# rajashree-srikanth/drone-sim-python

Hardware: NVIDIA B200
Metric: closed-loop aircraft-steps/s (higher is better)
Workload: dtype f64

## Files before the change

drone-sim-python_b200/csrc/d2dx_api.cu:

```cuda
#include <math.h>
#include <string.h>

#include "d2dx_device.cuh"
#include "d2dx_host.h"

namespace d2dx {

static thread_local char g_err[512] = "";

int set_error(int code, const char* fmt, ...) {
  va_list ap;
  va_start(ap, fmt);
  vsnprintf(g_err, sizeof(g_err), fmt, ap);
  va_end(ap);
  return code;
}

int rollout_resident_threads_per_sm();
int formation_resident_threads_per_sm();
int colloc_resident_threads_per_sm();

constexpr int kThreads = 128;
inline int grid_for(long n) { return (int)((n + kThreads - 1) / kThreads); }

// ... 82 lines not shown
  Ur[i] = r.u_phi; Ur[(size_t)n + i] = r.u_v;
  if (Xd) {
    Xd[i] = 0.0; Xd[(size_t)n + i] = 0.0; Xd[2 * (size_t)n + i] = r.psidot; Xd[3 * (size_t)n + i] = 0.0; Xd[4 * (size_t)n + i] = r.vadot;
  }
}

__global__ void __launch_bounds__(kThreads) dfff_control_kernel(const d2dx_traj_table tt, const double* __restrict__ X, double t,
                                                                 const double* __restrict__ W, const double* __restrict__ ac,
                                                                 const d2dx_dfff_gains g, double* __restrict__ U,
                                                                 double* __restrict__ Xr, double* __restrict__ K,
                                                                 double* __restrict__ care_state) {
  const int B = tt.n_traj, S = tt.n_seg;
  const int b = blockIdx.x * kThreads + threadIdx.x;
  if (b >= B) return;
  double te;
  const int seg = composite_locate(tt, b, t, te);
  auto P = [&](int k) { return tt.seg_par[(size_t)k * S + seg]; };
  FlatOut Y;
  segment_eval<false>(tt.seg_type[seg], P, te, Y, &tt);
  const AcPar a = load_ac(W, ac, B, b);
  double x[5];
  for (int k = 0; k < 5; ++k) x[k] = X[(size_t)k * B + b];
  const CareConst cc = care_const(g);
  CareState cs = {0.0, 1.0, 1.0, 0.0, 0.0};
  bool cold = true;
  if (care_state) {
    cs.C = care_state[b]; cs.S = care_state[B + b]; cs.al = care_state[2 * (size_t)B + b];
    cs.dth = care_state[3 * (size_t)B + b]; cs.dal = care_state[4 * (size_t)B + b];
    cold = !(cs.al > 0.0);
  }
  int flags = 0;
  RefCtl rc;
  double u_phi, u_v;
  make_ref(Y, a, ac[B + b], cc, cs, cold, flags, rc);
  feedback(rc, x, g, u_phi, u_v);
  U[b] = u_phi; U[(size_t)B + b] = u_v;
  if (Xr) { Xr[b] = rc.xr; Xr[(size_t)B + b] = rc.yr; Xr[2 * (size_t)B + b] = rc.psir; Xr[3 * (size_t)B + b] = rc.phir; Xr[4 * (size_t)B + b] = rc.var; }
  if (K) for (int k = 0; k < 6; ++k) K[(size_t)k * B + b] = rc.k[k];
  if (care_state) {
    care_state[b] = cs.C; care_state[B + b] = cs.S; care_state[2 * (size_t)B + b] = cold ? 0.0 : cs.al;
    care_state[3 * (size_t)B + b] = cs.dth; care_state[4 * (size_t)B + b] = cs.dal;
  }
}

__global__ void dfma_burn_kernel(int iters, double* sink) {
  double a[16];
  const double x = 1.0 + 1e-9 * threadIdx.x, y = 1e-12 * (blockIdx.x + 1);
#pragma unroll
  for (int k = 0; k < 16; ++k) a[k] = k * 0.5;
  for (int it = 0; it < iters; ++it) {
#pragma unroll
    for (int k = 0; k < 16; ++k) a[k] = fma(a[k], x, y);
  }
  double s = 0.0;
#pragma unroll
  for (int k = 0; k < 16; ++k) s += a[k];
  if (s == 123.456) *sink = s;
}

__global__ void math_probe_kernel(int n, const double* __restrict__ x, const double* __restrict__ y, double* __restrict__ out) {
  const int i = blockIdx.x * kThreads + threadIdx.x;
  if (i >= n) return;
  double s, c;
  fm::sincos(x[i], s, c);
// ... 160 lines not shown
```

drone-sim-python_b200/csrc/d2dx_device.cuh:

```cuda
#pragma once
#include <cuda_runtime.h>
#include <math.h>
#include <stdint.h>
#include <string.h>

#include "../../include/d2dx.h"
#include "d2dx_math.cuh"

namespace d2dx {

#ifdef D2DX_USE_LIBM
__device__ __forceinline__ void sincos_b(double x, double& s, double& c) { ::sincos(x, &s, &c); }
__device__ __forceinline__ void sincos_any(double x, double& s, double& c) { ::sincos(x, &s, &c); }
__device__ __forceinline__ double atan2_f(double y, double x) { return ::atan2(y, x); }
__device__ __forceinline__ double atan_f(double v) { return ::atan(v); }
__host__ __device__ __forceinline__ double sqrt_f(double v) { return ::sqrt(v); }
__host__ __device__ __forceinline__ double rsqrt_f(double v) { return 1.0 / ::sqrt(v); }
__host__ __device__ __forceinline__ double rcp_f(double v) { return 1.0 / v; }
__host__ __device__ __forceinline__ double div_f(double a, double b) { return a / b; }
#else
__device__ __forceinline__ void sincos_b(double x, double& s, double& c) { fm::sincos(x, s, c); }
struct SinCos { double s, c; };
static __device__ __noinline__ SinCos sincos_slow(double x) { SinCos r; ::sincos(x, &r.s, &r.c); return r; }
__device__ __forceinline__ void sincos_any(double x, double& s, double& c) {
// ... 332 lines not shown
  const double inv_va = rsqrt_f(va2), va = va2 * inv_va;
  r.x = Y.y0x; r.y = Y.y0y; r.va = va; r.inv_va = inv_va;
  r.psi = atan2_f(vay, vax);
  r.vadot = (vax * Y.y2x + vay * Y.y2y) * inv_va;
  const double num = Y.y2y * vax - Y.y2x * vay;
  r.psidot = num * inv_va * inv_va;
  r.z = num * inv_va * (1.0 / kG);
  r.phi = atan_f(r.z);
  r.u_phi = r.phi;
  r.u_v = tau_v * r.vadot + va;
  r.cpsi = vax * inv_va; r.spsi = vay * inv_va;
}

__host__ __device__ __forceinline__ int hi_word(double x) {
#ifdef __CUDA_ARCH__
  return __double2hiint(x);
#else
  long long b;
  memcpy(&b, &x, sizeof(b));
  return (int)(b >> 32);
#endif
}

struct CareState { double C, S, al, dth, dal; };

struct CareConst { double sq, q3, sr1, sr2, isr1, isr2; };

__host__ __device__ __forceinline__ CareConst care_const(const d2dx_dfff_gains& g) {
  CareConst c;
  c.sq = ::sqrt(g.q_pos); c.q3 = g.q_psi; c.sr1 = ::sqrt(g.r_phi); c.sr2 = ::sqrt(g.r_v);
  c.isr1 = 1.0 / c.sr1; c.isr2 = 1.0 / c.sr2;
  return c;
}

struct CareStep { double k1, ba, vc2, ve, k2, q3; };

__host__ __device__ __forceinline__ void care_residual(const CareStep& k, double C, double S, double al, double& be, double& F1, double& F2) {
  be = fma(k.k1, C, k.ba * al);
  F1 = fma(C, al, fma(S, be, fma(k.vc2, C, k.ve * S)));
  F2 = fma(al, al, fma(be, be, -fma(k.k2, S, k.q3)));
}

__host__ __device__ __forceinline__ void care_update(double& C, double& S, double& al, double dth, double dal) {
  const double Cn = fma(-S, dth, C), Sn = fma(C, dth, S);
  const double nrm = fma(-0.5, fma(Cn, Cn, Sn * Sn), 1.5);
  C = Cn * nrm; S = Sn * nrm; al += dal;
}

struct CareRoot { double C, S, al; bool conv; };
static __host__ __device__ __noinline__ CareRoot care_newton_loop_v(const CareStep k, double C, double S, double al, int max_it) {
  bool conv = false;
  for (int it = 0; it < max_it && !conv; ++it) {
    double be, F1, F2;
    care_residual(k, C, S, al, be, F1, F2);
    const double bt = -k.k1 * S;
    const double J11 = fma(-S, al, fma(C, be, fma(S, bt, fma(k.ve, C, -k.vc2 * S)))), J12 = fma(S, k.ba, C);
    const double J21 = 2.0 * fma(be, bt, -0.5 * k.k2 * C), J22 = 2.0 * fma(be, k.ba, al);
    const double idet = rcp_f(fma(J11, J22, -J12 * J21));
    const double dth = fma(J12, F2, -F1 * J22) * idet, dal = fma(J21, F1, -J11 * F2) * idet;
    const double Cn = C - S * dth, Sn = S + C * dth;
    const double nrm = rsqrt_f(fma(Cn, Cn, Sn * Sn));
    C = Cn * nrm; S = Sn * nrm; al += dal;
    conv = fabs(dth) < 3e-8 && fabs(dal) < 3e-8 * fabs(al);
  }
  CareRoot r;
  r.C = C; r.S = S; r.al = al; r.conv = conv;
  return r;
}
__host__ __device__ __forceinline__ bool care_newton_loop(const CareStep& k, double& C, double& S, double& al, int max_it) {
  const CareRoot r = care_newton_loop_v(k, C, S, al, max_it);
  C = r.C; S = r.S; al = r.al;
  return r.conv;
}

__host__ __device__ __forceinline__ bool care_gain(const CareConst& cc, double v, double c1, double e, CareState& st, bool cold, double* K0) {
  const double c1q = c1 * cc.sq;
  CareStep k;
  k.k1 = c1q * cc.isr2; k.ba = e * cc.isr2; k.vc2 = v * cc.sr2; k.ve = v * e; k.k2 = 2.0 * v * c1q; k.q3 = cc.q3;
  const double C0 = st.C, S0 = st.S, al0 = st.al;
  double C = C0, S = S0, al = al0;
  care_update(C, S, al, st.dth, st.dal);
  double be_, F1, F2;
  care_residual(k, C, S, al, be_, F1, F2);
  const double bt = -k.k1 * S;
  const double J11 = fma(-S, al, fma(C, be_, fma(S, bt, fma(k.ve, C, -k.vc2 * S)))), J12 = fma(S, k.ba, C);
  const double J21 = 2.0 * fma(be_, bt, -0.5 * k.k2 * C), J22 = 2.0 * fma(be_, k.ba, al);
  const double idet = rcp_f(fma(J11, J22, -J12 * J21));
  const double i11 = J22 * idet, i12 = -J12 * idet, i21 = -J21 * idet, i22 = J11 * idet;
  double dth = -fma(i11, F1, i12 * F2), dal = -fma(i21, F1, i22 * F2);
  care_update(C, S, al, dth, dal);
  care_residual(k, C, S, al, be_, F1, F2);
  dth = -fma(i11, F1, i12 * F2); dal = -fma(i21, F1, i22 * F2);
  care_update(C, S, al, dth, dal);
  bool ok = !cold && (hi_word(dth) & 0x7fffffff) < 0x3E601B2B && fabs(dal) < 3e-8 * fabs(al) && hi_word(S) > 0 && hi_word(al) > 0;
  if (!ok) {
    if (!cold) {
      C = C0; S = S0; al = al0;
      ok = care_newton_loop(k, C, S, al, 40) && S > 0.0 && al > 0.0;
    }
    if (!ok) { C = 0.0; S = 1.0; al = sqrt_f(cc.q3 + k.k2); ok = care_newton_loop(k, C, S, al, 60); }
  }
  st.dth = fma(C0, S, -S0 * C); st.dal = al - al0;
  if (cold || !((hi_word(st.dth) & 0x7fffffff) < 0x3F947AE1 && fabs(st.dal) < 0.02 * al)) { st.dth = 0.0; st.dal = 0.0; }
  st.C = C; st.S = S; st.al = al;
  const double be = fma(k.k1, C, k.ba * al);
  K0[0] = cc.sq * C * cc.isr1; K0[1] = cc.sq * S * cc.isr1; K0[2] = al * cc.isr1;
  K0[3] = cc.sq * S * cc.isr2; K0[4] = -cc.sq * C * cc.isr2; K0[5] = be * cc.isr2;
  return ok;
}

struct RefCtl { double xr, yr, psir, phir, var, uphi, uv, k[6]; };

__device__ __forceinline__ void make_ref(const FlatOut& Y, const AcPar& a, double tau_v, const CareConst& cc, CareState& cs,
                                         bool& cold, int& flags, RefCtl& r) {
  FlatState fr;
  flatness(Y, a.wx, a.wy, tau_v, fr);
  const double z2 = fr.z * fr.z;
  const double c1 = cc.sr1 * (2.0 + z2) * rcp_f(kG * fr.inv_va * (1.0 + z2));
  const double e = kG * fr.inv_va * fr.inv_va * fr.z * c1;
  double K0[6];
  if (care_gain(cc, fr.va, c1, e, cs, cold, K0)) cold = false;
  else { flags |= 2; cold = true; }
  r.xr = fr.x; r.yr = fr.y; r.psir = fr.psi; r.phir = fr.phi; r.var = fr.va; r.uphi = fr.u_phi; r.uv = fr.u_v;
#pragma unroll
  for (int m = 0; m < 2; ++m) {
    r.k[3 * m + 0] = K0[3 * m] * fr.cpsi - K0[3 * m + 1] * fr.spsi;
    r.k[3 * m + 1] = K0[3 * m] * fr.spsi + K0[3 * m + 1] * fr.cpsi;
    r.k[3 * m + 2] = K0[3 * m + 2];
  }
}

__device__ __forceinline__ void feedback(const RefCtl& r, const double* X, const d2dx_dfff_gains& g, double& u_phi, double& u_v) {
  const double ex = clip_sym(X[0] - r.xr, g.err_sat[0]);
  const double ey = clip_sym(X[1] - r.yr, g.err_sat[1]);
  const double ep = clip_sym(wrap_pi(X[2] - r.psir), g.err_sat[2]);
  u_phi = clip(r.uphi - fma(r.k[0], ex, fma(r.k[1], ey, r.k[2] * ep)), g.u_lo[0], g.u_hi[0]);
  u_v = clip(r.uv - fma(r.k[3], ex, fma(r.k[4], ey, r.k[5] * ep)), g.u_lo[1], g.u_hi[1]);
}

__device__ __forceinline__ void gvf_control(double px, double py, double psi, double v, double cx, double cy,
                                            double r, double ke, double kd, double& U, double& U1, double& U2) {
  const double dx = px - cx, dy = py - cy;
  const double e = (dx * dx + dy * dy) - r * r;
  const double nx = 2.0 * dx, ny = 2.0 * dy;
  double s, c;
  sincos_b(psi, s, c);
  const double pdx = v * c, pdy = v * s;
  const double tx = ny, ty = -nx;
  const double qx = tx - ke * e * nx, qy = ty - ke * e * ny;
  const double inrm = rsqrt_f(qx * qx + qy * qy);
  const double qnx = qx * inrm, qny = qy * inrm;
  const double ox = qny, oy = -qnx;
// ... 38 lines not shown
```

drone-sim-python_b200/csrc/d2dx_lqr5.cuh:

```cuda
#pragma once
#include "d2dx_device.cuh"

namespace d2dx {

struct Lqr5State { double C, S, p23, p24, p33, p34, p44; };

struct Lqr5Par { double v, a, b, itp, itv, s1, s2, i1, i2, sq, q3, q4, q5; };

__host__ __device__ __forceinline__ bool solve6(double (&J)[6][6], double (&F)[6], double (&d)[6]) {
  constexpr int perm[6] = {2, 0, 3, 1, 4, 5};
  double A[6][7];
#pragma unroll
  for (int i = 0; i < 6; ++i) {
#pragma unroll
    for (int j = 0; j < 6; ++j) A[i][j] = J[perm[i]][j];
    A[i][6] = -F[perm[i]];
  }
  bool ok = true;
#pragma unroll
  for (int k = 0; k < 6; ++k) {
    double amax = fabs(A[k][k]);
#pragma unroll
    for (int j = k + 1; j < 6; ++j) amax = fabs(A[k][j]) > amax ? fabs(A[k][j]) : amax;
    ok = ok && (fabs(A[k][k]) > 1e-9 * amax);
// ... 50 lines not shown
    J[3][4] = (sq * S + P.b * y2) * P.i2 * ia - x2 * P.i1; J[4][4] = -(P.itp + P.itv) - (x3 * P.i1 + y4 * P.i2); J[5][4] = -2.0 * x4 * P.i1;
    J[0][5] = 0.0; J[1][5] = 0.0; J[2][5] = sq * C * P.i2; J[3][5] = -y2 * P.i2; J[4][5] = -y3 * P.i2; J[5][5] = -2.0 * (P.itv + y4 * P.i2);
    if (!solve6(J, F, d)) return false;
    const double Cn = C - S * d[0], Sn = S + C * d[0];
    const double nrm = rsqrt_f(Cn * Cn + Sn * Sn);
    u.C = Cn * nrm; u.S = Sn * nrm;
    u.p23 += d[1]; u.p24 += d[2]; u.p33 += d[3]; u.p34 += d[4]; u.p44 += d[5];
    const double scale = fabs(u.p23) + fabs(u.p24) + fabs(u.p33) + fabs(u.p34) + fabs(u.p44);
    const double step = fabs(d[1]) + fabs(d[2]) + fabs(d[3]) + fabs(d[4]) + fabs(d[5]);
    if (fabs(d[0]) < 3e-8 && step < 3e-8 * scale) return true;
  }
  return false;
}

__host__ __device__ inline bool lqr5_gain(const Lqr5Par& P, double sr1, double sr2, double tau_phi, double tau_v, double r1, double r2,
                                          Lqr5State& st, double* Kp) {
  bool ok = false;
  if (st.p23 > 0.0) {
    Lqr5State w = st;
    ok = lqr5_newton(P, w, 12) && w.S > 0.0 && w.p23 > 0.0;
    if (ok) st = w;
  }
  if (!ok) {
    CareConst cc; cc.sq = P.sq; cc.q3 = P.q3; cc.sr1 = sr1; cc.sr2 = sr2; cc.isr1 = 1.0 / sr1; cc.isr2 = 1.0 / sr2;
    CareState c3 = {0.0, 1.0, 1.0, 0.0, 0.0};
    double K0[6];
    const double c1 = sr1 * rcp_f(P.a), e = P.b * c1;
    care_gain(cc, P.v, c1, e, c3, true, K0);
    const double al3 = K0[2] * sr1, be3 = K0[5] * sr2;
    st.C = c3.C; st.S = c3.S;
    st.p23 = P.s1 * al3; st.p24 = P.s2 * be3;
    st.p33 = tau_phi * (P.a * st.p23 + 0.5 * P.q4);
    st.p44 = tau_v * (P.s2 * P.sq * st.S + P.b * st.p24 + 0.5 * P.q5);
    st.p34 = (P.a * st.p24 + P.s1 * P.sq * st.C + P.b * st.p23) * rcp_f(P.itp + P.itv);
    ok = lqr5_newton(P, st, 40);
  }
  const double f1 = 1.0 / (tau_phi * r1), f2 = 1.0 / (tau_v * r2);
  Kp[0] = P.s1 * P.sq * st.C * f1; Kp[1] = P.s1 * P.sq * st.S * f1;
  Kp[5] = P.s2 * P.sq * st.S * f2; Kp[6] = -P.s2 * P.sq * st.C * f2;
  Kp[2] = st.p23 * f1; Kp[3] = st.p33 * f1; Kp[4] = st.p34 * f1;
  Kp[7] = st.p24 * f2; Kp[8] = st.p34 * f2; Kp[9] = st.p44 * f2;
  return ok;
}

}
```

drone-sim-python_b200/csrc/d2dx_rollout.cu:

```cuda
#include "d2dx_device.cuh"
#include "d2dx_host.h"

namespace d2dx {

constexpr int kRolloutThreads = 128;
#ifndef D2DX_ROLLOUT_MIN_BLOCKS
#define D2DX_ROLLOUT_MIN_BLOCKS 4
#endif

struct RolloutArgs {
  d2dx_scenarios s;
  d2dx_rollout_out o;
  d2dx_dfff_gains g;
  CareConst cc;
  const double* time;
  int i_begin, i_end, nsub, final_control;
};

__device__ __forceinline__ void tma_load_1d(void* smem_dst, const void* gmem_src, uint32_t bytes, uint64_t* bar) {
  const uint32_t dst = static_cast<uint32_t>(__cvta_generic_to_shared(smem_dst));
  const uint32_t mb = static_cast<uint32_t>(__cvta_generic_to_shared(bar));
  asm volatile("cp.async.bulk.shared::cluster.global.mbarrier::complete_tx::bytes [%0], [%1], %2, [%3];"
               :: "r"(dst), "l"(gmem_src), "r"(bytes), "r"(mb) : "memory");
}
// ... 38 lines not shown
      }
      mbar_wait(&bar, 0);
    } else {
      for (int k = 0; k < kRows; ++k) spar[k][tid] = tt.seg_par[(size_t)k * S + b];
    }
    cur_seg = b;
  }
  auto P = [&](int k) { return spar[k][tid]; };

  spar[D2DX_SEG_NPAR + 0][tid] = a.s.wind[b]; spar[D2DX_SEG_NPAR + 1][tid] = a.s.wind[B + b];
  spar[D2DX_SEG_NPAR + 2][tid] = -1.0 / a.s.ac[b]; spar[D2DX_SEG_NPAR + 3][tid] = -1.0 / a.s.ac[B + b];
  spar[D2DX_SEG_NPAR + 4][tid] = a.s.ac[B + b];
  auto load_ac = [&]() {
    AcPar ap;
    ap.wx = spar[D2DX_SEG_NPAR + 0][tid]; ap.wy = spar[D2DX_SEG_NPAR + 1][tid];
    ap.n_inv_tau_phi = spar[D2DX_SEG_NPAR + 2][tid]; ap.n_inv_tau_v = spar[D2DX_SEG_NPAR + 3][tid];
    return ap;
  };
  double X[5];
#pragma unroll
  for (int k = 0; k < 5; ++k) X[k] = a.s.X0[(size_t)k * B + b];

  const CareConst& cc = a.cc;
  CareState cs = {0.0, 1.0, 1.0, 0.0, 0.0};
  bool cold = true;
  if (a.o.care_state) {
    cs.C = a.o.care_state[b]; cs.S = a.o.care_state[B + b]; cs.al = a.o.care_state[2 * (size_t)B + b];
    cs.dth = a.o.care_state[3 * (size_t)B + b]; cs.dal = a.o.care_state[4 * (size_t)B + b];
    cold = !(cs.al > 0.0);
  }
  int flags = 0;
  double sum_sq = 0.0, max_sq = 0.0;

  int ev = 0, ev_end = 0, ev_next = 0x7fffffff;
  if (a.s.pert_begin) {
    ev = a.s.pert_begin[b]; ev_end = a.s.pert_begin[b + 1];
    while (ev < ev_end && a.s.pert_step[ev] <= a.i_begin) ++ev;
    if (ev < ev_end) ev_next = a.s.pert_step[ev];
  }

  auto reference_at = [&](double t, RefCtl& r) {
    FlatOut Y;
    if (UNIFORM >= 0) {
      segment_eval<false>(UNIFORM, P, t, Y);
    } else {
      double te;
      const int seg = composite_locate(tt, b, t, te);
      if (seg != cur_seg) {
        cur_seg = seg; seg_type = tt.seg_type[seg];
        for (int k = 0; k < D2DX_SEG_NPAR; ++k) spar[k][tid] = tt.seg_par[(size_t)k * S + seg];
      }
      segment_eval<false>(seg_type, P, te, Y, &tt);
    }
    make_ref(Y, load_ac(), spar[D2DX_SEG_NPAR + 4][tid], cc, cs, cold, flags, r);
  };

  const int log_every = a.o.log_every > 0 ? a.o.log_every : 1;
  const int n_samples = a.i_end - a.i_begin + (a.final_control ? 1 : 0);
  double t = a.time[a.i_begin];
  int log_in = (log_every - a.i_begin % log_every) % log_every;
  for (int n = 0; n < n_samples; ++n) {
    const int i = a.i_begin + n;
    RefCtl ref;
    reference_at(t, ref);
    double u_phi, u_v;
    feedback(ref, X, a.g, u_phi, u_v);
    const double ex = X[0] - ref.xr, ey = X[1] - ref.yr, d2 = ex * ex + ey * ey;
    sum_sq += d2; max_sq = __double_as_longlong(d2) > __double_as_longlong(max_sq) ? d2 : max_sq;
    const bool log_now = LOGGING && log_in == 0;
    log_in = log_now ? log_every - 1 : log_in - 1;
    if (log_now && active) {
      const size_t row = (size_t)(i / log_every);
      if (a.o.X_log) {
#pragma unroll
        for (int k = 0; k < 5; ++k) a.o.X_log[(row * 5 + k) * B + b] = X[k];
      }
      if (a.o.U_log) { a.o.U_log[(row * 2) * B + b] = u_phi; a.o.U_log[(row * 2 + 1) * B + b] = u_v; }
// ... 7 lines not shown
      }
    }
    if (i == a.i_end) break;
    const double t1 = a.time[i + 1];
    if (a.nsub == 1) rk4_step<true>(load_ac(), X, u_phi, u_v, t1 - t, 1);
    else rk4_step(load_ac(), X, u_phi, u_v, t1 - t, a.nsub);
    t = t1;
    if (i + 1 == ev_next) {
#pragma unroll
      for (int k = 0; k < 5; ++k) X[k] += a.s.pert_dx[(size_t)k * a.s.n_events + ev];
      ++ev;
      ev_next = ev < ev_end ? a.s.pert_step[ev] : 0x7fffffff;
    }
  }
  if (!isfinite(X[0] + X[1] + X[2] + X[3] + X[4])) flags |= 1;

  if (active) {
#pragma unroll
    for (int k = 0; k < 5; ++k) a.o.X_final[(size_t)k * B + b] = X[k];
    if (a.o.sum_sq_err) a.o.sum_sq_err[b] += sum_sq;
    if (a.o.max_err) a.o.max_err[b] = fmax(a.o.max_err[b], sqrt(max_sq));
    if (a.o.flags) a.o.flags[b] |= flags;
    if (a.o.care_state) {
      a.o.care_state[b] = cs.C; a.o.care_state[B + b] = cs.S;
      a.o.care_state[2 * (size_t)B + b] = cold ? 0.0 : cs.al;
      a.o.care_state[3 * (size_t)B + b] = cs.dth; a.o.care_state[4 * (size_t)B + b] = cs.dal;
    }
  }
  if (a.o.pop_stats) {
    const double ws = warp_sum(active ? sum_sq : 0.0);
    const double wm = warp_max(active ? sqrt(max_sq) : 0.0);
    if ((tid & 31) == 0) { atomicAdd(a.o.pop_stats, ws); atomic_max_double(a.o.pop_stats + 1, wm); }
  }
}

template <int UNIFORM>
static int launch_rollout(const RolloutArgs& a, bool logging, cudaStream_t st) {
  const int grid = (a.s.B + kRolloutThreads - 1) / kRolloutThreads;
  const bool logref = a.o.Xr_log || a.o.K_log;
  if (logref) rollout_dfff_kernel<UNIFORM, true, true><<<grid, kRolloutThreads, 0, st>>>(a);
  else if (logging) rollout_dfff_kernel<UNIFORM, true, false><<<grid, kRolloutThreads, 0, st>>>(a);
  else rollout_dfff_kernel<UNIFORM, false, false><<<grid, kRolloutThreads, 0, st>>>(a);
  D2DX_LAUNCH_CHECK("rollout_dfff_kernel");
  return D2DX_OK;
}

int rollout_resident_threads_per_sm() {
  int nb = 0;
  cudaOccupancyMaxActiveBlocksPerMultiprocessor(&nb, rollout_dfff_kernel<D2DX_SEG_CIRCLE, false, false>, kRolloutThreads, 0);
// ... 38 lines not shown
```

drone-sim-python_b200/csrc/host_check.cu:

```cuda
#include <vector>

#include "d2dx_ddp.cuh"
#include "d2dx_lqr5.cuh"

using namespace d2dx;

extern "C" {

int d2dx_host_care_gain(const double* qr4 , double v, double phi, int cold, double* state5, double* K0) {
  d2dx_dfff_gains g;
  g.q_pos = qr4[0]; g.q_psi = qr4[1]; g.r_phi = qr4[2]; g.r_v = qr4[3];
  const CareConst cc = care_const(g);
  const double z = tan(phi), z2 = z * z, inv_va = 1.0 / v;
  const double c1 = cc.sr1 * (2.0 + z2) * rcp_f(kG * inv_va * (1.0 + z2));
  const double e = kG * inv_va * inv_va * z * c1;
  CareState st = {state5[0], state5[1], state5[2], state5[3], state5[4]};
  const bool ok = care_gain(cc, v, c1, e, st, cold != 0, K0);
  state5[0] = st.C; state5[1] = st.S; state5[2] = st.al; state5[3] = st.dth; state5[4] = st.dal;
  return ok ? 1 : 0;
}

int d2dx_host_lqr5_gain(const double* q5, const double* r2, double v, double phi, double tau_phi, double tau_v, double* state7, double* Kp) {
  const double z = tan(phi), z2 = z * z, inv_va = 1.0 / v;
  Lqr5Par P;
  P.v = v;
  P.a = kG * inv_va * (1.0 + z2) * rcp_f(2.0 + z2);
  P.b = kG * inv_va * inv_va * z;
  P.itp = 1.0 / tau_phi; P.itv = 1.0 / tau_v;
  P.sq = ::sqrt(q5[0]); P.q3 = q5[2]; P.q4 = q5[3]; P.q5 = q5[4];
  const double sr1 = ::sqrt(r2[0]), sr2 = ::sqrt(r2[1]);
  P.s1 = tau_phi * sr1; P.s2 = tau_v * sr2; P.i1 = 1.0 / P.s1; P.i2 = 1.0 / P.s2;
  Lqr5State st = {state7[0], state7[1], state7[2], state7[3], state7[4], state7[5], state7[6]};
  const bool ok = lqr5_gain(P, sr1, sr2, tau_phi, tau_v, r2[0], r2[1], st, Kp);
  state7[0] = st.C; state7[1] = st.S; state7[2] = st.p23; state7[3] = st.p24; state7[4] = st.p33; state7[5] = st.p34; state7[6] = st.p44;
  return ok ? 1 : 0;
}

int d2dx_host_ddp_solve(const double* prob9, int n_obs, const double* obs, const double* bounds4, const double* box5, const double* z0,
                        const double* zt, const d2dx_ddp_options* o, double* u, double* xs, double* info) {
  DdpProblem P;
  P.N = (int)prob9[0]; P.h = prob9[1]; P.wx = prob9[2]; P.wy = prob9[3]; P.vsp = prob9[4]; P.kv = prob9[5]; P.kb = prob9[6];
  P.kobs = prob9[7]; P.obs_kind = (int)prob9[8]; P.n_obs = n_obs;
// ... 29 lines not shown
```

drone-sim-python_b200/d2d_b200/_lib.py:

```python
import ctypes as C
import os

_HERE = os.path.dirname(os.path.abspath(__file__))
LIB_PATH = os.environ.get("D2DX_LIB") or os.path.join(_HERE, "libd2dx.so")

SEG_LINE, SEG_CIRCLE, SEG_SLALOM, SEG_POLY, SEG_SI_LINE, SEG_TABLE, SEG_SI_CIRCLE = range(7)
SEG_NPAR = 17
JAC_COMPACT, JAC_OPTY_DENSE = 0, 1
EVAL_RESIDUAL, EVAL_JAC, EVAL_COST, EVAL_GRAD = 1, 2, 4, 8
EVAL_ALL = 15
MAX_OBSTACLES = 16
PEER_MAX_WORLD, IPC_HANDLE_BYTES = 16, 64

c_dp = C.c_void_p


class TrajTable(C.Structure):
    _fields_ = [("n_traj", C.c_int32), ("n_seg", C.c_int32),
                ("first_seg", c_dp), ("n_segs", c_dp), ("traj_t0", c_dp), ("traj_dur", c_dp),
                ("seg_type", c_dp), ("seg_end", c_dp), ("seg_par", c_dp), ("uniform_type", C.c_int32),
                ("n_tab", C.c_int32), ("tab_time", c_dp), ("tab_x", c_dp), ("tab_y", c_dp), ("tab_vx", c_dp), ("tab_vy", c_dp)]


class DfffGains(C.Structure):
    _fields_ = [("q_pos", C.c_double), ("q_psi", C.c_double), ("r_phi", C.c_double), ("r_v", C.c_double),
                ("err_sat", C.c_double * 5), ("u_lo", C.c_double * 2), ("u_hi", C.c_double * 2)]


class Scenarios(C.Structure):
    _fields_ = [("B", C.c_int32), ("X0", c_dp), ("wind", c_dp), ("ac", c_dp), ("traj", TrajTable),
                ("pert_begin", c_dp), ("pert_step", c_dp), ("pert_dx", c_dp), ("n_events", C.c_int32)]


class RolloutOut(C.Structure):
    _fields_ = [("log_every", C.c_int32), ("X_log", c_dp), ("U_log", c_dp), ("Xr_log", c_dp), ("K_log", c_dp),
# ... 135 lines not shown
```

drone-sim-python_b200/d2d_b200/guidance.py:

```python
import numpy as np

from . import trajectory as ddt
from .dynamic import Aircraft
from .engine import get_engine


def norm_mpi_pi(v):
    eng = get_engine()
    a = np.asarray(v, dtype=np.float64)
    out = eng.norm_mpi_pi(eng.to_device(np.ascontiguousarray(a.reshape(-1)))).cpu().numpy().reshape(a.shape)
    return float(out) if a.ndim == 0 else out


class WindField:

    def __init__(self, w=[0., 0.]):
        self.w = w

    def sample(self, t, loc):
        return self.w

    def summarize(self):
        return f"{self.w} m/s"

# ... 8 lines not shown
        n = len(Yb)
        Yd = eng.to_device(np.ascontiguousarray(Yb.reshape(n, 8).T))
        Wd = eng.to_device(np.ascontiguousarray(np.broadcast_to(np.asarray(W, dtype=np.float64).reshape(-1, 2), (n, 2)).T))
        acd = eng.to_device(np.ascontiguousarray(np.broadcast_to(np.array([[ac.tau_phi], [ac.tau_v]]), (2, n))))
        Xr, Ur, Xd = (a.cpu().numpy().T for a in eng.flatness(Yd, Wd, acd))
        return (Xr[0], Ur[0], Xd[0]) if single else (Xr, Ur, Xd)


class DFFFController:

    def __init__(self, traj, ac, wind):
        self.traj, self.ac, self.wind = traj, ac, wind
        self.dt = 0.01
        self.time = np.arange(0, traj.duration, self.dt)
        self.carrot, self.ref_pos = [0, 0], [0, 0]
        self.Xref, self.K = [], []
        self._table = None
        self._care = None

    def get(self, X, t):
        eng = get_engine()
        if self._table is None:
            self._table = eng.table(ddt.pack([self.traj]))
            self._care = eng.zeros(5, 1)
        W = np.asarray(self.wind.sample(t, None), dtype=np.float64).reshape(2, 1)
        acd = eng.to_device(np.array([[self.ac.tau_phi], [self.ac.tau_v]]))
        Xd = eng.to_device(np.asarray(X, dtype=np.float64).reshape(5, 1))
        U, Xr, K = eng.dfff_control(self._table, Xd, t, eng.to_device(W), acd, care_state=self._care)
        self.Xref.append(Xr.cpu().numpy()[:, 0])
        K5 = np.zeros((2, 5))
        K5[:, :3] = K.cpu().numpy()[:, 0].reshape(2, 3)
        self.K.append(K5)
        return U.cpu().numpy()[:, 0]


class DCFController:

    def get(self, n_ac, B, c, p, z_des, kr):
        eng = get_engine()
        z_des = np.asarray(z_des, dtype=np.float64)
        B = np.asarray(B, dtype=np.float64).reshape(n_ac, -1)
        c = np.asarray(c, dtype=np.float64)
        if c.shape != (n_ac, 2):
            raise ValueError(f"operands could not be broadcast together: p is (2,{n_ac}), c.T is {c.T.shape} "
                             "(c must be (n_ac, 2), cf. d2d/guidance.py:106)")
        pd = eng.to_device(np.ascontiguousarray(np.asarray(p, dtype=np.float64).reshape(2, n_ac)))
        cd = eng.to_device(np.ascontiguousarray(c.T))
# ... 75 lines not shown
```

drone-sim-python_b200/d2d_b200/simulation.py:

```python
import numpy as np
import torch

from . import trajectory as ddt
from .dynamic import Aircraft
from .engine import get_engine
from .guidance import DFFFController, PurePursuitControler, WindField


def _perts_csr(eng, perts_list, T):
    begin, steps, dxs = [0], [], []
    for p in perts_list:
        if p is not None:
            p = np.asarray(p, dtype=np.float64)
            rows = np.nonzero(np.any(p != 0., axis=1))[0]
            rows = rows[rows >= 1]
            steps += list(rows); dxs += [p[r] for r in rows]
        begin.append(len(steps))
    if not steps:
        return None
    return (eng.to_device(np.asarray(begin, np.int32)), eng.to_device(np.asarray(steps, np.int32)),
            eng.to_device(np.ascontiguousarray(np.asarray(dxs, np.float64).T)))


class RolloutResult:
# ... 41 lines not shown
    T = len(time)
    X0 = np.asarray(X0, dtype=np.float64).reshape(-1, 5)
    B = len(X0)
    if group_by_family and isinstance(trajs, (list, tuple)) and B >= 256 and len(trajs) == B:
        fams = [_family(tr) for tr in trajs]
        if len(set(fams)) > 1:
            return _rollout_by_family(time, trajs, wind, X0, perts, tau_phi, tau_v, fams, nsub=nsub, log_every=log_every, log_ref=log_ref,
                                      final_control=final_control, gains=gains, engine=eng, chunk_steps=chunk_steps, return_log=return_log)
    packed = ddt.pack(trajs)
    if packed.n_traj != B:
        raise ValueError(f"{packed.n_traj} trajectories for {B} initial states")
    tab = eng.table(packed)
    wind = np.broadcast_to(np.asarray(wind, dtype=np.float64).reshape(-1, 2), (B, 2))
    ac = np.stack([np.broadcast_to(np.asarray(tau_phi, dtype=np.float64), (B,)), np.broadcast_to(np.asarray(tau_v, dtype=np.float64), (B,))])
    X0d, Wd, acd, td = eng.to_device(np.ascontiguousarray(X0.T)), eng.to_device(np.ascontiguousarray(wind.T)), eng.to_device(ac), eng.to_device(time)
    pd = _perts_csr(eng, perts, T) if perts is not None else None
    n_rows = (T - 1) // log_every + 1
    X_log = eng.empty(n_rows, 5, B) if return_log else None
    U_log = eng.empty(n_rows, 2, B) if return_log else None
    Xr_log = eng.empty(n_rows, 5, B) if (log_ref and return_log) else None
    K_log = eng.empty(n_rows, 6, B) if (log_ref and return_log) else None
    sum_sq, max_err = eng.zeros(B), eng.zeros(B)
    flags = eng.zeros(B, dtype=torch.int32)
    care = eng.zeros(5, B)
    pop = eng.zeros(2)
    X_final = eng.empty(5, B)
    chunk = chunk_steps or (T - 1)
    i, Xc = 0, X0d
    while True:
        j = min(i + chunk, T - 1)
        last = j == T - 1
        eng.rollout_dfff(tab, Xc, Wd, acd, td, i, j, nsub=nsub, final_control=(final_control and last), gains=gains,
                         log_every=log_every, X_log=X_log, U_log=U_log, Xr_log=Xr_log, K_log=K_log, X_final=X_final,
                         sum_sq_err=sum_sq, max_err=max_err, flags=flags, care_state=care, pop_stats=pop, perts=pd)
        if last:
            break
        i, Xc = j, X_final
    if return_log and not final_control and (T - 1) % log_every == 0:
        X_log[n_rows - 1] = X_final
        for t_ in (U_log, Xr_log, K_log):
            if t_ is not None:
                t_[n_rows - 1].zero_()
    res = RolloutResult()
    res.time_log = time[::log_every]
    res.X_final = X_final.cpu().numpy().T
    res.sum_sq_err, res.max_err, res.flags = sum_sq.cpu().numpy(), max_err.cpu().numpy(), flags.cpu().numpy()
    res.pop_sum_sq_err, res.pop_max_err = (float(v) for v in pop.cpu().numpy())
# ... 126 lines not shown
        self.seg_type = int(seg_type)
        self.n_par_rows = {_lib.SEG_CIRCLE: 6, _lib.SEG_LINE: 5}.get(self.seg_type, _lib.SEG_NPAR)
        pin = lambda *shape, dtype=torch.float64: torch.empty(*shape, dtype=dtype).pin_memory()
        B = self.B
        self.h_X0, self.h_wind, self.h_ac, self.h_par = pin(5, B), pin(2, B), pin(2, B), pin(self.n_par_rows, B)
        self.h_Xf, self.h_ss, self.h_mx, self.h_flags = pin(5, B), pin(B), pin(B), pin(B, dtype=torch.int32)
        self.h_pop = pin(2)
        self.host_log, self.log_u = host_log, log_u
        self.h_Xlog = pin(self.n_rows, 5, B) if host_log else None
        self.h_Ulog = pin(self.n_rows, 2, B) if (host_log and log_u and host_log_u) else None
        self.d_X0, self.d_wind, self.d_ac = eng.empty(5, B), eng.empty(2, B), eng.empty(2, B)
        par = eng.zeros(_lib.SEG_NPAR, B)
        ar = np.arange(B, dtype=np.int32)
        self.table = eng.table(PackedTrajectories(ar, np.ones(B, np.int32), np.zeros(B), np.zeros(B),
                                                  np.full(B, self.seg_type, np.int32), np.zeros(B), np.zeros((_lib.SEG_NPAR, B)),
                                                  self.seg_type))
        self.d_par = self.table.t["seg_par"]
        del par
        self.d_time = eng.to_device(self.time)
        self.d_Xlog = eng.empty(self.n_rows, 5, B)
        self.d_Ulog = eng.empty(self.n_rows, 2, B) if log_u else None
        self.d_Xf, self.d_Xa, self.d_Xb = eng.empty(5, B), eng.empty(5, B), eng.empty(5, B)
        self.d_ss, self.d_mx, self.d_flags = eng.zeros(B), eng.zeros(B), eng.zeros(B, dtype=torch.int32)
        self.d_care, self.d_pop = eng.zeros(5, B), eng.zeros(2)
        steps = self.T - 1
        per = max(self.log_every, ((steps + n_chunks - 1) // n_chunks + self.log_every - 1) // self.log_every * self.log_every)
        self.bounds = list(range(0, steps, per)) + [steps]
        self.copy_stream = torch.cuda.Stream(device=eng.device)
        self.h2d_bytes = sum(t.numel() * t.element_size() for t in (self.h_X0, self.h_wind, self.h_ac, self.h_par))
        self.d2h_bytes = sum(t.numel() * t.element_size() for t in (self.h_Xf, self.h_ss, self.h_mx, self.h_flags, self.h_pop)) + \
            sum(t.numel() * t.element_size() for t in (self.h_Xlog, self.h_Ulog) if t is not None)
        self.launches_per_run = len(self.bounds) - 1

    def set_inputs(self, par_rows, wind, X0, tau_phi=0.01, tau_v=1.):
        self.h_par.numpy()[...] = par_rows
        self.h_wind.numpy()[...] = np.asarray(wind, dtype=np.float64).T
        self.h_X0.numpy()[...] = np.asarray(X0, dtype=np.float64).T
        self.h_ac.numpy()[0], self.h_ac.numpy()[1] = tau_phi, tau_v

    def upload(self):
        self.d_X0.copy_(self.h_X0, non_blocking=True); self.d_wind.copy_(self.h_wind, non_blocking=True)
        self.d_ac.copy_(self.h_ac, non_blocking=True); self.d_par[:self.n_par_rows].copy_(self.h_par, non_blocking=True)

    def _sweep(self, copy_logs):
        eng = self.eng
        self.d_ss.zero_(); self.d_mx.zero_(); self.d_flags.zero_(); self.d_care.zero_(); self.d_pop.zero_()
        cur = torch.cuda.current_stream(eng.device)
# ... 39 lines not shown
```

include/d2dx.h:

```cpp
#ifndef D2DX_H
#define D2DX_H

#include <stdint.h>

#ifdef __cplusplus
extern "C" {
#endif

#define D2DX_VERSION 103

enum { D2DX_OK = 0, D2DX_EINVAL = 1, D2DX_ECUDA = 2, D2DX_EUNSUPPORTED = 3 };

typedef struct d2dx_handle d2dx_handle;

int d2dx_version(void);
const char* d2dx_last_error(void);
int d2dx_create(int device, d2dx_handle** out);
int d2dx_destroy(d2dx_handle* h);
int d2dx_device_info(d2dx_handle* h, int32_t* what_host4);

enum {
  D2DX_SEG_LINE = 0,
  D2DX_SEG_CIRCLE = 1,
  D2DX_SEG_SLALOM = 2,
  D2DX_SEG_POLY = 3,
  D2DX_SEG_SI_LINE = 4,
  D2DX_SEG_TABLE = 5,
  D2DX_SEG_SI_CIRCLE = 6
};
#define D2DX_SEG_NPAR 17

typedef struct {
// ... 16 lines not shown
} d2dx_traj_table;

int d2dx_traj_eval(d2dx_handle* h, const d2dx_traj_table* tt, int32_t nT, const double* time,
                   double* Y, void* stream);

int d2dx_cont_dyn(d2dx_handle* h, int32_t n, const double* X, const double* U, const double* W,
                  const double* ac, double* Xdot, void* stream);
int d2dx_disc_dyn(d2dx_handle* h, int32_t n, const double* X, const double* U, const double* W,
                  const double* ac, double dt, int32_t nsub, double* Xnext, void* stream);
int d2dx_cont_jac(d2dx_handle* h, int32_t n, const double* Xr, const double* ac, double* A,
                  double* Bm, void* stream);
int d2dx_flatness(d2dx_handle* h, int32_t n, const double* Ys, const double* W, const double* ac,
                  double* Xr, double* Ur, double* Xrdot, void* stream);

int d2dx_norm_mpi_pi(d2dx_handle* h, int32_t n, const double* v, double* out, void* stream);

typedef struct {
  double q_pos, q_psi;
  double r_phi, r_v;
  double err_sat[5];
  double u_lo[2], u_hi[2];
} d2dx_dfff_gains;
int d2dx_dfff_default_gains(d2dx_dfff_gains* g_host);

int d2dx_dfff_control(d2dx_handle* h, const d2dx_traj_table* tt, const double* X, double t,
                      const double* W, const double* ac, const d2dx_dfff_gains* gains_host,
                      double* U, double* Xr, double* K, double* care_state, void* stream);

typedef struct {
  int32_t B;
  const double* X0;
  const double* wind;
  const double* ac;
  d2dx_traj_table traj;
  const int32_t* pert_begin;
  const int32_t* pert_step;
  const double* pert_dx;
  int32_t n_events;
} d2dx_scenarios;

typedef struct {
  int32_t log_every;
  double* X_log;
  double* U_log;
  double* Xr_log;
  double* K_log;
// ... 191 lines not shown
```

Measured before the change: 32.80 billion.

## Use quadratic warm-start extrapolation and single Newton step in CARE gain

The CARE warm-start state grows from 5 to 9 rows, keeping three past increments of the angle and alpha so the next root guess is extrapolated quadratically instead of linearly. With the better guess, the fast path does one Newton correction instead of two, and its acceptance tolerance on the step is loosened. It also precomputes products of the gain constants and rotates C/S once before forming the gains, which trims per-step double-precision work. The risks are more register and state traffic per aircraft, and more frequent fallback to the slow Newton loop if the extrapolated guess is poor.

Result: faster. 33.82 billion, median of 6 (+3.1%).

```diff
diff --git a/drone-sim-python_b200/csrc/d2dx_api.cu b/drone-sim-python_b200/csrc/d2dx_api.cu
--- a/drone-sim-python_b200/csrc/d2dx_api.cu
+++ b/drone-sim-python_b200/csrc/d2dx_api.cu
@@ -128,24 +128,20 @@
   double x[5];
   for (int k = 0; k < 5; ++k) x[k] = X[(size_t)k * B + b];
   const CareConst cc = care_const(g);
-  CareState cs = {0.0, 1.0, 1.0, 0.0, 0.0};
-  bool cold = true;
-  if (care_state) {
-    cs.C = care_state[b]; cs.S = care_state[B + b]; cs.al = care_state[2 * (size_t)B + b];
-    cs.dth = care_state[3 * (size_t)B + b]; cs.dal = care_state[4 * (size_t)B + b];
-    cold = !(cs.al > 0.0);
-  }
+  double cs[kCareState] = {};
+  if (care_state)
+    for (int k = 0; k < kCareState; ++k) cs[k] = care_state[k * (size_t)B + b];
+  bool cold = !(cs[2] > 0.0);
   int flags = 0;
   RefCtl rc;
   double u_phi, u_v;
-  make_ref(Y, a, ac[B + b], cc, cs, cold, flags, rc);
+  make_ref(Y, a, ac[B + b], cc, ArrayState{cs}, cold, flags, rc);
   feedback(rc, x, g, u_phi, u_v);
   U[b] = u_phi; U[(size_t)B + b] = u_v;
   if (Xr) { Xr[b] = rc.xr; Xr[(size_t)B + b] = rc.yr; Xr[2 * (size_t)B + b] = rc.psir; Xr[3 * (size_t)B + b] = rc.phir; Xr[4 * (size_t)B + b] = rc.var; }
   if (K) for (int k = 0; k < 6; ++k) K[(size_t)k * B + b] = rc.k[k];
   if (care_state) {
-    care_state[b] = cs.C; care_state[B + b] = cs.S; care_state[2 * (size_t)B + b] = cold ? 0.0 : cs.al;
-    care_state[3 * (size_t)B + b] = cs.dth; care_state[4 * (size_t)B + b] = cs.dal;
+    for (int k = 0; k < kCareState; ++k) care_state[k * (size_t)B + b] = (k == 2 && cold) ? 0.0 : cs[k];
   }
 }
 
diff --git a/drone-sim-python_b200/csrc/d2dx_device.cuh b/drone-sim-python_b200/csrc/d2dx_device.cuh
--- a/drone-sim-python_b200/csrc/d2dx_device.cuh
+++ b/drone-sim-python_b200/csrc/d2dx_device.cuh
@@ -378,15 +378,23 @@
 #endif
 }
 
-struct CareState { double C, S, al, dth, dal; };
-
-struct CareConst { double sq, q3, sr1, sr2, isr1, isr2; };
-
+constexpr int kCareState = D2DX_CARE_STATE_ROWS;
+struct CareSol { double C, S, al, be; };
+struct ArrayState {
+  double* p;
+  __host__ __device__ double& operator()(int k) const { return p[k]; }
+};
+
+struct CareConst { double q3, sr1, sr2, isr1, isr2, sq2, sq_isr1, sq_isr2; };
+
+__host__ __device__ __forceinline__ CareConst care_const(double sq, double q3, double sr1, double sr2) {
+  CareConst c;
+  c.q3 = q3; c.sr1 = sr1; c.sr2 = sr2; c.isr1 = 1.0 / sr1; c.isr2 = 1.0 / sr2;
+  c.sq2 = 2.0 * sq; c.sq_isr1 = sq * c.isr1; c.sq_isr2 = sq * c.isr2;
+  return c;
+}
 __host__ __device__ __forceinline__ CareConst care_const(const d2dx_dfff_gains& g) {
-  CareConst c;
-  c.sq = ::sqrt(g.q_pos); c.q3 = g.q_psi; c.sr1 = ::sqrt(g.r_phi); c.sr2 = ::sqrt(g.r_v);
-  c.isr1 = 1.0 / c.sr1; c.isr2 = 1.0 / c.sr2;
-  return c;
+  return care_const(::sqrt(g.q_pos), g.q_psi, ::sqrt(g.r_phi), ::sqrt(g.r_v));
 }
 
 struct CareStep { double k1, ba, vc2, ve, k2, q3; };
@@ -429,61 +437,65 @@
   return r.conv;
 }
 
-__host__ __device__ __forceinline__ bool care_gain(const CareConst& cc, double v, double c1, double e, CareState& st, bool cold, double* K0) {
-  const double c1q = c1 * cc.sq;
+constexpr int kCareStepTolHi = 0x3E800000;
+constexpr int kCareStepTolExp = 23 << 20;
+enum { CARE_FAILED = 0, CARE_LOOP = 1, CARE_FAST = 2 };
+
+template <class State>
+__host__ __device__ __forceinline__ int care_gain(const CareConst& cc, double v, double c1, double e, State&& st, bool cold, CareSol& sol) {
   CareStep k;
-  k.k1 = c1q * cc.isr2; k.ba = e * cc.isr2; k.vc2 = v * cc.sr2; k.ve = v * e; k.k2 = 2.0 * v * c1q; k.q3 = cc.q3;
-  const double C0 = st.C, S0 = st.S, al0 = st.al;
-  double C = C0, S = S0, al = al0;
-  care_update(C, S, al, st.dth, st.dal);
+  k.k1 = c1 * cc.sq_isr2; k.ba = e * cc.isr2; k.vc2 = v * cc.sr2; k.ve = v * e; k.k2 = v * c1 * cc.sq2; k.q3 = cc.q3;
+  const double th1 = st(3), th2 = st(4), th3 = st(5), al1 = st(6), al2 = st(7), al3 = st(8);
+  st(4) = th1; st(5) = th2; st(7) = al1; st(8) = al2;
+  const double p = fma(3.0, th1 - th2, th3), cp = fma(-0.5 * p, p, 1.0);
+  double C = fma(st(0), cp, -st(1) * p), S = fma(st(1), cp, st(0) * p), al = st(2) + fma(3.0, al1 - al2, al3);
   double be_, F1, F2;
   care_residual(k, C, S, al, be_, F1, F2);
   const double bt = -k.k1 * S;
   const double J11 = fma(-S, al, fma(C, be_, fma(S, bt, fma(k.ve, C, -k.vc2 * S)))), J12 = fma(S, k.ba, C);
   const double J21 = 2.0 * fma(be_, bt, -0.5 * k.k2 * C), J22 = 2.0 * fma(be_, k.ba, al);
   const double idet = rcp_f(fma(J11, J22, -J12 * J21));
-  const double i11 = J22 * idet, i12 = -J12 * idet, i21 = -J21 * idet, i22 = J11 * idet;
-  double dth = -fma(i11, F1, i12 * F2), dal = -fma(i21, F1, i22 * F2);
+  const double dth = fma(J12, F2, -F1 * J22) * idet, dal = fma(J21, F1, -J11 * F2) * idet;
   care_update(C, S, al, dth, dal);
-  care_residual(k, C, S, al, be_, F1, F2);
-  dth = -fma(i11, F1, i12 * F2); dal = -fma(i21, F1, i22 * F2);
-  care_update(C, S, al, dth, dal);
-  bool ok = !cold && (hi_word(dth) & 0x7fffffff) < 0x3E601B2B && fabs(dal) < 3e-8 * fabs(al) && hi_word(S) > 0 && hi_word(al) > 0;
-  if (!ok) {
+  const int hal = hi_word(al);
+  int res = (!cold && (hi_word(dth) & 0x7fffffff) < kCareStepTolHi && (hi_word(dal) & 0x7fffffff) + kCareStepTolExp < hal &&
+             hi_word(S) > 0 && hal > 0) ? CARE_FAST : CARE_FAILED;
+  if (res == CARE_FAILED) {
     if (!cold) {
-      C = C0; S = S0; al = al0;
-      ok = care_newton_loop(k, C, S, al, 40) && S > 0.0 && al > 0.0;
+      C = st(0); S = st(1); al = st(2);
+      if (care_newton_loop(k, C, S, al, 40) && S > 0.0 && al > 0.0) res = CARE_LOOP;
     }
-    if (!ok) { C = 0.0; S = 1.0; al = sqrt_f(cc.q3 + k.k2); ok = care_newton_loop(k, C, S, al, 60); }
-  }
-  st.dth = fma(C0, S, -S0 * C); st.dal = al - al0;
-  if (cold || !((hi_word(st.dth) & 0x7fffffff) < 0x3F947AE1 && fabs(st.dal) < 0.02 * al)) { st.dth = 0.0; st.dal = 0.0; }
-  st.C = C; st.S = S; st.al = al;
-  const double be = fma(k.k1, C, k.ba * al);
-  K0[0] = cc.sq * C * cc.isr1; K0[1] = cc.sq * S * cc.isr1; K0[2] = al * cc.isr1;
-  K0[3] = cc.sq * S * cc.isr2; K0[4] = -cc.sq * C * cc.isr2; K0[5] = be * cc.isr2;
-  return ok;
+    if (res == CARE_FAILED) {
+      C = 0.0; S = 1.0; al = sqrt_f(cc.q3 + k.k2);
+      if (care_newton_loop(k, C, S, al, 60)) res = CARE_LOOP;
+    }
+  }
+  const double nth = fma(st(0), S, -st(1) * C), nal = al - st(2);
+  const bool keep = !cold && (hi_word(nth) & 0x7fffffff) < 0x3F947AE1 && (hi_word(nal) & 0x7fffffff) + (6 << 20) < hi_word(al);
+  st(0) = C; st(1) = S; st(2) = al;
+  st(3) = keep ? nth : 0.0; st(6) = keep ? nal : 0.0;
+  if (!keep) { st(4) = 0.0; st(5) = 0.0; st(7) = 0.0; st(8) = 0.0; }
+  sol.C = C; sol.S = S; sol.al = al; sol.be = fma(k.k1, C, k.ba * al);
+  return res;
 }
 
 struct RefCtl { double xr, yr, psir, phir, var, uphi, uv, k[6]; };
 
-__device__ __forceinline__ void make_ref(const FlatOut& Y, const AcPar& a, double tau_v, const CareConst& cc, CareState& cs,
+template <class State>
+__device__ __forceinline__ void make_ref(const FlatOut& Y, const AcPar& a, double tau_v, const CareConst& cc, State&& care,
                                          bool& cold, int& flags, RefCtl& r) {
   FlatState fr;
   flatness(Y, a.wx, a.wy, tau_v, fr);
   const double z2 = fr.z * fr.z;
   const double c1 = cc.sr1 * (2.0 + z2) * rcp_f(kG * fr.inv_va * (1.0 + z2));
   const double e = kG * fr.inv_va * fr.inv_va * fr.z * c1;
-  double K0[6];
-  if (care_gain(cc, fr.va, c1, e, cs, cold, K0)) cold = false;
+  CareSol cs;
+  if (care_gain(cc, fr.va, c1, e, care, cold, cs) != CARE_FAILED) cold = false;
   else { flags |= 2; cold = true; }
   r.xr = fr.x; r.yr = fr.y; r.psir = fr.psi; r.phir = fr.phi; r.var = fr.va; r.uphi = fr.u_phi; r.uv = fr.u_v;
-#pragma unroll
-  for (int m = 0; m < 2; ++m) {
-    r.k[3 * m + 0] = K0[3 * m] * fr.cpsi - K0[3 * m + 1] * fr.spsi;
-    r.k[3 * m + 1] = K0[3 * m] * fr.spsi + K0[3 * m + 1] * fr.cpsi;
-    r.k[3 * m + 2] = K0[3 * m + 2];
-  }
+  const double Cw = fma(cs.C, fr.cpsi, -cs.S * fr.spsi), Sw = fma(cs.C, fr.spsi, cs.S * fr.cpsi);
+  r.k[0] = cc.sq_isr1 * Cw; r.k[1] = cc.sq_isr1 * Sw; r.k[2] = cs.al * cc.isr1;
+  r.k[3] = cc.sq_isr2 * Sw; r.k[4] = -cc.sq_isr2 * Cw; r.k[5] = cs.be * cc.isr2;
 }
 
 __device__ __forceinline__ void feedback(const RefCtl& r, const double* X, const d2dx_dfff_gains& g, double& u_phi, double& u_v) {
diff --git a/drone-sim-python_b200/csrc/d2dx_lqr5.cuh b/drone-sim-python_b200/csrc/d2dx_lqr5.cuh
--- a/drone-sim-python_b200/csrc/d2dx_lqr5.cuh
+++ b/drone-sim-python_b200/csrc/d2dx_lqr5.cuh
@@ -96,12 +96,12 @@
     if (ok) st = w;
   }
   if (!ok) {
-    CareConst cc; cc.sq = P.sq; cc.q3 = P.q3; cc.sr1 = sr1; cc.sr2 = sr2; cc.isr1 = 1.0 / sr1; cc.isr2 = 1.0 / sr2;
-    CareState c3 = {0.0, 1.0, 1.0, 0.0, 0.0};
-    double K0[6];
+    const CareConst cc = care_const(P.sq, P.q3, sr1, sr2);
+    double s3[kCareState] = {};
+    CareSol c3;
     const double c1 = sr1 * rcp_f(P.a), e = P.b * c1;
-    care_gain(cc, P.v, c1, e, c3, true, K0);
-    const double al3 = K0[2] * sr1, be3 = K0[5] * sr2;
+    care_gain(cc, P.v, c1, e, ArrayState{s3}, true, c3);
+    const double al3 = c3.al, be3 = c3.be;
     st.C = c3.C; st.S = c3.S;
     st.p23 = P.s1 * al3; st.p24 = P.s2 * be3;
     st.p33 = tau_phi * (P.a * st.p23 + 0.5 * P.q4);
diff --git a/drone-sim-python_b200/csrc/d2dx_rollout.cu b/drone-sim-python_b200/csrc/d2dx_rollout.cu
--- a/drone-sim-python_b200/csrc/d2dx_rollout.cu
+++ b/drone-sim-python_b200/csrc/d2dx_rollout.cu
@@ -84,13 +84,10 @@
   for (int k = 0; k < 5; ++k) X[k] = a.s.X0[(size_t)k * B + b];
 
   const CareConst& cc = a.cc;
-  CareState cs = {0.0, 1.0, 1.0, 0.0, 0.0};
-  bool cold = true;
-  if (a.o.care_state) {
-    cs.C = a.o.care_state[b]; cs.S = a.o.care_state[B + b]; cs.al = a.o.care_state[2 * (size_t)B + b];
-    cs.dth = a.o.care_state[3 * (size_t)B + b]; cs.dal = a.o.care_state[4 * (size_t)B + b];
-    cold = !(cs.al > 0.0);
-  }
+  double care[kCareState];
+#pragma unroll
+  for (int k = 0; k < kCareState; ++k) care[k] = a.o.care_state ? a.o.care_state[k * (size_t)B + b] : 0.0;
+  bool cold = !(care[2] > 0.0);
   int flags = 0;
   double sum_sq = 0.0, max_sq = 0.0;
 
@@ -114,7 +111,7 @@
       }
       segment_eval<false>(seg_type, P, te, Y, &tt);
     }
-    make_ref(Y, load_ac(), spar[D2DX_SEG_NPAR + 4][tid], cc, cs, cold, flags, r);
+    make_ref(Y, load_ac(), spar[D2DX_SEG_NPAR + 4][tid], cc, ArrayState{care}, cold, flags, r);
   };
 
   const int log_every = a.o.log_every > 0 ? a.o.log_every : 1;
@@ -168,9 +165,8 @@
     if (a.o.max_err) a.o.max_err[b] = fmax(a.o.max_err[b], sqrt(max_sq));
     if (a.o.flags) a.o.flags[b] |= flags;
     if (a.o.care_state) {
-      a.o.care_state[b] = cs.C; a.o.care_state[B + b] = cs.S;
-      a.o.care_state[2 * (size_t)B + b] = cold ? 0.0 : cs.al;
-      a.o.care_state[3 * (size_t)B + b] = cs.dth; a.o.care_state[4 * (size_t)B + b] = cs.dal;
+#pragma unroll
+      for (int k = 0; k < kCareState; ++k) a.o.care_state[k * (size_t)B + b] = (k == 2 && cold) ? 0.0 : care[k];
     }
   }
   if (a.o.pop_stats) {
diff --git a/drone-sim-python_b200/csrc/host_check.cu b/drone-sim-python_b200/csrc/host_check.cu
--- a/drone-sim-python_b200/csrc/host_check.cu
+++ b/drone-sim-python_b200/csrc/host_check.cu
@@ -7,17 +7,29 @@
 
 extern "C" {
 
-int d2dx_host_care_gain(const double* qr4 , double v, double phi, int cold, double* state5, double* K0) {
+static int care_gain_host(const double* qr4, double v, double phi, int cold, double* state9, double* K0) {
   d2dx_dfff_gains g;
   g.q_pos = qr4[0]; g.q_psi = qr4[1]; g.r_phi = qr4[2]; g.r_v = qr4[3];
   const CareConst cc = care_const(g);
   const double z = tan(phi), z2 = z * z, inv_va = 1.0 / v;
   const double c1 = cc.sr1 * (2.0 + z2) * rcp_f(kG * inv_va * (1.0 + z2));
   const double e = kG * inv_va * inv_va * z * c1;
-  CareState st = {state5[0], state5[1], state5[2], state5[3], state5[4]};
-  const bool ok = care_gain(cc, v, c1, e, st, cold != 0, K0);
-  state5[0] = st.C; state5[1] = st.S; state5[2] = st.al; state5[3] = st.dth; state5[4] = st.dal;
-  return ok ? 1 : 0;
+  CareSol sol;
+  const int res = care_gain(cc, v, c1, e, ArrayState{state9}, cold != 0, sol);
+  K0[0] = cc.sq_isr1 * sol.C; K0[1] = cc.sq_isr1 * sol.S; K0[2] = sol.al * cc.isr1;
+  K0[3] = cc.sq_isr2 * sol.S; K0[4] = -cc.sq_isr2 * sol.C; K0[5] = sol.be * cc.isr2;
+  return res;
+}
+
+int d2dx_host_care_gain9(const double* qr4 , double v, double phi, int cold, double* state9, double* K0) {
+  return care_gain_host(qr4, v, phi, cold, state9, K0);
+}
+
+int d2dx_host_care_gain(const double* qr4, double v, double phi, int cold, double* state5, double* K0) {
+  double s9[9] = {state5[0], state5[1], state5[2], state5[3], state5[3], state5[3], state5[4], state5[4], state5[4]};
+  const int res = care_gain_host(qr4, v, phi, cold, s9, K0);
+  state5[0] = s9[0]; state5[1] = s9[1]; state5[2] = s9[2]; state5[3] = s9[3]; state5[4] = s9[6];
+  return res != CARE_FAILED ? 1 : 0;
 }
 
 int d2dx_host_lqr5_gain(const double* q5, const double* r2, double v, double phi, double tau_phi, double tau_v, double* state7, double* Kp) {
diff --git a/drone-sim-python_b200/d2d_b200/_lib.py b/drone-sim-python_b200/d2d_b200/_lib.py
--- a/drone-sim-python_b200/d2d_b200/_lib.py
+++ b/drone-sim-python_b200/d2d_b200/_lib.py
@@ -11,6 +11,7 @@
 EVAL_ALL = 15
 MAX_OBSTACLES = 16
 PEER_MAX_WORLD, IPC_HANDLE_BYTES = 16, 64
+CARE_STATE_ROWS = 9
 
 c_dp = C.c_void_p
 
diff --git a/drone-sim-python_b200/d2d_b200/guidance.py b/drone-sim-python_b200/d2d_b200/guidance.py
--- a/drone-sim-python_b200/d2d_b200/guidance.py
+++ b/drone-sim-python_b200/d2d_b200/guidance.py
@@ -54,7 +54,8 @@
         eng = get_engine()
         if self._table is None:
             self._table = eng.table(ddt.pack([self.traj]))
-            self._care = eng.zeros(5, 1)
+            from . import _lib
+            self._care = eng.zeros(_lib.CARE_STATE_ROWS, 1)
         W = np.asarray(self.wind.sample(t, None), dtype=np.float64).reshape(2, 1)
         acd = eng.to_device(np.array([[self.ac.tau_phi], [self.ac.tau_v]]))
         Xd = eng.to_device(np.asarray(X, dtype=np.float64).reshape(5, 1))
diff --git a/drone-sim-python_b200/d2d_b200/simulation.py b/drone-sim-python_b200/d2d_b200/simulation.py
--- a/drone-sim-python_b200/d2d_b200/simulation.py
+++ b/drone-sim-python_b200/d2d_b200/simulation.py
@@ -87,7 +87,8 @@
     K_log = eng.empty(n_rows, 6, B) if (log_ref and return_log) else None
     sum_sq, max_err = eng.zeros(B), eng.zeros(B)
     flags = eng.zeros(B, dtype=torch.int32)
-    care = eng.zeros(5, B)
+    from . import _lib
+    care = eng.zeros(_lib.CARE_STATE_ROWS, B)
     pop = eng.zeros(2)
     X_final = eng.empty(5, B)
     chunk = chunk_steps or (T - 1)
@@ -260,7 +261,7 @@
         self.d_Ulog = eng.empty(self.n_rows, 2, B) if log_u else None
         self.d_Xf, self.d_Xa, self.d_Xb = eng.empty(5, B), eng.empty(5, B), eng.empty(5, B)
         self.d_ss, self.d_mx, self.d_flags = eng.zeros(B), eng.zeros(B), eng.zeros(B, dtype=torch.int32)
-        self.d_care, self.d_pop = eng.zeros(5, B), eng.zeros(2)
+        self.d_care, self.d_pop = eng.zeros(_lib.CARE_STATE_ROWS, B), eng.zeros(2)
         steps = self.T - 1
         per = max(self.log_every, ((steps + n_chunks - 1) // n_chunks + self.log_every - 1) // self.log_every * self.log_every)
         self.bounds = list(range(0, steps, per)) + [steps]
diff --git a/include/d2dx.h b/include/d2dx.h
--- a/include/d2dx.h
+++ b/include/d2dx.h
@@ -7,7 +7,7 @@
 extern "C" {
 #endif
 
-#define D2DX_VERSION 103
+#define D2DX_VERSION 104
 
 enum { D2DX_OK = 0, D2DX_EINVAL = 1, D2DX_ECUDA = 2, D2DX_EUNSUPPORTED = 3 };
 
@@ -70,6 +70,8 @@
   double u_lo[2], u_hi[2];
 } d2dx_dfff_gains;
 int d2dx_dfff_default_gains(d2dx_dfff_gains* g_host);
+
+#define D2DX_CARE_STATE_ROWS 9
 
 int d2dx_dfff_control(d2dx_handle* h, const d2dx_traj_table* tt, const double* X, double t,
                       const double* W, const double* ac, const d2dx_dfff_gains* gains_host,
```
